# bindingflare/bling

Measured on AMD Instinct MI355X. Metric: Mrays/sec (primary+secondary), cornell-box 1024x1024 64spp at 1/2/4/8 GPU, higher is better.
Workload: dtype f32

## Files before the change

bling_amd/_ffi.py:

```python
from __future__ import annotations

import ctypes as C
import os

_HERE = os.path.dirname(os.path.abspath(__file__))
LIBDIR = os.path.join(_HERE, "_lib")

c_f32p = C.POINTER(C.c_float)
c_u32p = C.POINTER(C.c_uint32)


PASS_TRAVERSAL_STATS = 1
PASS_KERNEL_TIMING = 2
PASS_TILE_IMAGES = 4
PASS_REGION_EVENTS = 8
PASS_NO_MIS_CULL = 16


class PassParams(C.Structure):
    _fields_ = [("seed", C.c_uint32), ("pass_index", C.c_uint32), ("shard_rank", C.c_int32),
                ("shard_world", C.c_int32), ("tile_stride", C.c_int32), ("chunk_paths", C.c_int32),
                ("flags", C.c_uint32), ("tiles_device", C.c_void_p), ("tiles_capacity", C.c_uint64)]


# ... 67 lines not shown
        lib.bling_host_summary.restype = C.c_char_p
        lib.bling_host_free.argtypes = [C.c_void_p]
        lib.bling_host_config.argtypes = [C.c_void_p, C.POINTER(RenderConfig)]
        lib.bling_host_filter_size.argtypes = [C.c_void_p, c_f32p]
        lib.bling_host_filter_table.argtypes = [C.c_void_p, c_f32p]
        lib.bling_host_counts.argtypes = [C.c_void_p, c_u32p]
        lib.bling_host_last_error.restype = C.c_char_p
        lib.bling_host_film_to_rgb.argtypes = [c_f32p, C.c_int, C.c_int, c_f32p]
        lib.bling_host_film_splat_to_rgb.argtypes = [c_f32p, c_f32p, C.c_float, C.c_int, C.c_int, c_f32p]
        lib.bling_host_light.argtypes = [C.c_void_p, C.POINTER(LightTracer)]
        lib.bling_host_write_hdr.argtypes = [C.c_char_p, c_f32p, C.c_int, C.c_int]
        lib.bling_host_write_hdr.restype = C.c_int
        lib.bling_host_rgb_pixels.argtypes = [c_f32p, C.c_int, C.c_int, C.POINTER(C.c_uint8)]
        lib.bling_host_write_png.argtypes = [C.c_char_p, c_f32p, C.c_int, C.c_int]
        lib.bling_host_write_png.restype = C.c_int
        _host = lib
    return _host


HIP_SYMBOLS = ["bling_create", "bling_scene_upload", "bling_scene_validate", "bling_render_pass", "bling_render_pass_device",
               "bling_trace", "bling_trace_device", "bling_sample_li", "bling_sample_li_vertices", "bling_pass_tile_layout",
               "bling_film_add_tiles", "bling_film_add_shards", "bling_sppm_pass", "bling_sppm_pixel_stats", "bling_sppm_reset",
               "bling_render", "bling_debug_stream_bytes", "bling_debug_scene_info", "bling_debug_mis_culled", "bling_debug_set_mis_cull", "bling_debug_sppm_hitpoints", "bling_debug_sppm_buckets",
               "bling_light_pass", "bling_debug_light_records", "bling_destroy", "bling_last_error", "bling_version"]


class Progress(C.Structure):
    _fields_ = [("kind", C.c_int32), ("pass_", C.c_int32), ("film", C.POINTER(C.c_float)), ("splat_weight", C.c_float),
                ("pass_stats", C.POINTER(Stats)), ("region", C.c_int32 * 4)]


PROGRESS_STARTED, PROGRESS_SAMPLES_ADDED, PROGRESS_REGION_STARTED, PROGRESS_PASS_DONE = 0, 1, 2, 3
ProgressFn = C.CFUNCTYPE(C.c_int, C.c_void_p, C.POINTER(Progress))
STREAM_NAMES = "queue,hit,meta,org,dir,mdir,mhit,occ,fac,cf,T,L,Tn,lsc,bsc,sh_o,sh_d,result,qflag".split(",")


def hip() -> C.CDLL:
    global _hip
    if _hip is None:
        var = os.environ.get("BLING_HIP_VARIANT", "")
        path = os.path.join(LIBDIR, f"libbling_hip_{var}.so" if var else "libbling_hip.so")
        if not os.path.exists(path):
            raise OSError(f"{path} missing: run `make` (the HIP core has no CPU fallback)")
        lib = C.CDLL(path)
        lib.bling_create.argtypes = [C.POINTER(C.c_int), C.c_int, C.POINTER(C.c_void_p)]
        lib.bling_create.restype = C.c_int
        lib.bling_scene_upload.argtypes = [C.c_void_p, C.c_void_p]
        lib.bling_scene_upload.restype = C.c_int
        if hasattr(lib, "bling_scene_validate"):
            lib.bling_scene_validate.argtypes = [C.c_void_p]
            lib.bling_scene_validate.restype = C.c_int
        lib.bling_render_pass.argtypes = [C.c_void_p, C.POINTER(PassParams), c_f32p, C.POINTER(Stats)]
        lib.bling_render_pass.restype = C.c_int
        lib.bling_render_pass_device.argtypes = [C.c_void_p, C.POINTER(PassParams), C.c_void_p, C.POINTER(Stats)]
        lib.bling_render_pass_device.restype = C.c_int
        lib.bling_pass_tile_layout.argtypes = [C.c_void_p, C.POINTER(PassParams), C.POINTER(C.c_int32),
                                               C.POINTER(C.c_size_t), C.POINTER(C.c_int32), C.POINTER(C.c_int32)]
        lib.bling_pass_tile_layout.restype = C.c_int
        lib.bling_film_add_tiles.argtypes = [C.c_void_p, C.POINTER(PassParams), C.c_void_p, C.c_void_p]
        lib.bling_film_add_tiles.restype = C.c_int
        lib.bling_film_add_shards.argtypes = [C.c_void_p, C.POINTER(PassParams), C.POINTER(C.c_void_p), C.c_void_p]
        lib.bling_film_add_shards.restype = C.c_int
        lib.bling_trace.argtypes = [C.c_void_p, c_f32p, C.c_size_t, C.c_int, c_f32p, c_u32p, c_f32p]
        lib.bling_trace.restype = C.c_int
        lib.bling_trace_device.argtypes = [C.c_void_p, C.c_void_p, C.c_size_t, C.c_int, C.c_void_p, C.c_void_p,
                                           C.c_void_p, C.c_int, C.POINTER(C.c_double)]
        lib.bling_trace_device.restype = C.c_int
# ... 46 lines not shown
```

bling_amd/csrc/core/core_internal.h:

```cpp
#pragma once
#include <hip/hip_runtime.h>

#include <algorithm>
#include <type_traits>
#include <cstdio>
#include <cstring>
#include <memory>
#include <stdexcept>
#include <string>
#include <vector>

#include "../../../include/bling.h"
#include "../common/scene_features.h"
#include "bvh_build.h"
#include "wavefront.h"
#include "sppm.h"
#include "light_tracer.h"

namespace bcore {
using namespace bd;

struct HipError : std::runtime_error { using std::runtime_error::runtime_error; };

#define HIPCHK(x)                                                                        \
  do {                                                                                   \
    hipError_t e_ = (x);                                                                 \
    if (e_ != hipSuccess) throw HipError(std::string(#x) + ": " + hipGetErrorString(e_)); \
  } while (0)

template <class T>
struct DBuf {
  T* p = nullptr;
  size_t n = 0;
  DBuf() = default;
  DBuf(const DBuf&) = delete;
  DBuf& operator=(const DBuf&) = delete;
  void alloc(size_t count) {
    free();
    if (count == 0) return;
    HIPCHK(hipMalloc(&p, count * sizeof(T)));
    n = count;
  }
  void upload(const T* h, size_t count) {
    alloc(count);
    if (count) HIPCHK(hipMemcpy(p, h, count * sizeof(T), hipMemcpyHostToDevice));
  }
  void free() { if (p) { (void)hipFree(p); p = nullptr; n = 0; } }
  ~DBuf() { free(); }
};


constexpr uint64_t kSetBytes = 9 * 16 + 8 + 4 + 64 + 64;
constexpr uint64_t kSetSpectraBytes = 3 * 64;
constexpr uint64_t kPathFixedBytes = 16 + 8 + 6 * 4 + 1 + 4 + 2 * 4;
constexpr uint64_t kDlSlotBytes = 16 + 16 + 64;
constexpr int kMaxDlDepth = 16;

struct SppmState {
  bool ready = false;
  uint32_t hp_cap = 0, items_cap = 0, n_stats = 0, nth = 0, n_tiles = 0, n_ext = 0;
  DBuf<float4> hp_pos, hp_hit, hp_o, hp_d, hp_f, result;
  DBuf<Bsdf> hp_bsdf;
  DBuf<float2> img;
  DBuf<uint32_t> hp_count, cnt, bstart, bcur, items;
  DBuf<float> r2, nacc, splat, film, kd_mr, kd_c;
  DBuf<unsigned long long> hp_key;
  DBuf<SppmGrid> grid;
  DBuf<unsigned long long> ctr;
  DBuf<TileDesc> tiles;
  void free_all() {
    for (auto* b : {&hp_pos, &hp_hit, &hp_o, &hp_d, &hp_f, &result}) b->free();
    img.free(); hp_bsdf.free();
    for (auto* b : {&hp_count, &cnt, &bstart, &bcur, &items}) b->free();
    for (auto* b : {&r2, &nacc, &splat, &film, &kd_mr, &kd_c}) b->free();
    hp_key.free(); grid.free(); ctr.free(); tiles.free();
    ready = false; hp_cap = items_cap = 0;
  }
};

struct LightState {
  DBuf<float> splat;
  DBuf<unsigned long long> ctr;
  DBuf<uint4> rec;
  DBuf<uint32_t> rec_count;
  void free_all() { splat.free(); ctr.free(); rec.free(); rec_count.free(); }
};

}

using namespace bd;
using namespace bcore;

struct bling_ctx {
  using WaveState = bd::WaveState;
  int device = 0;
  hipStream_t stream = nullptr;
  bool has_scene = false;
  DevScene S{};
  DBuf<float4> nodes, tri_geo, pkt;
  DBuf<float4> leaf_geo;
  DBuf<uint32_t> refs;
  DBuf<float> tri_normals;
  DBuf<float4> tri_frame;
  DBuf<uint8_t> tri_has_n;
  DBuf<int32_t> tri_material, tri_prim, shape_prim;
  DBuf<DevShape> shapes;
  DBuf<bling_material> materials;
  DBuf<bling_texture> textures;
  DBuf<bling_scalar_texture> stex;
  DBuf<bling_light> lights;
  DBuf<bling_image> images;
  std::vector<std::unique_ptr<DBuf<float>>> light_arrays;
  uint32_t cap = 0;
  struct SetBufs {
    DBuf<float4> org, dir, hit, mdir, fac, cf, sh_o, sh_d, T, Tn, L, lsc, bsc;
    DBuf<uint4> meta;
    DBuf<float2> mhit;
    DBuf<uint32_t> occ;
    void alloc(uint32_t n, bool spectra) {
      for (auto* b : {&org, &dir, &hit, &mdir, &fac, &cf, &sh_o, &sh_d}) b->alloc(n);
      meta.alloc(n); mhit.alloc(n); occ.alloc(n);
      T.alloc((size_t)4 * n); L.alloc((size_t)4 * n);
      if (spectra) { Tn.alloc((size_t)4 * n); lsc.alloc((size_t)4 * n); bsc.alloc((size_t)4 * n); }
      else { Tn.free(); lsc.free(); bsc.free(); }
    }
    void free() {
      for (auto* b : {&org, &dir, &hit, &mdir, &fac, &cf, &sh_o, &sh_d, &T, &Tn, &L, &lsc, &bsc}) b->free();
      meta.free(); mhit.free(); occ.free();
    }
    PathSet view() const {
      return PathSet{org.p, dir.p, hit.p, meta.p, mdir.p, mhit.p, occ.p, fac.p, cf.p, sh_o.p, sh_d.p,
                     T.p, Tn.p, L.p, lsc.p, bsc.p};
    }
  } set[2];
  bool sets_spectra = false, sets_two = false;
  DBuf<float4> corg, dl_org, dl_dir, dl_T;
  DBuf<uint32_t> dl_mask;
  int dl_levels = 0;
  DBuf<float4> result;
  DBuf<float2> img;
  DBuf<uint32_t> qmem, qcount, blk;
  DBuf<float> march;
  DBuf<uint8_t> qflag;
  DBuf<TileDesc> tiles_dev;
  DBuf<Counters> counters;
  uint64_t mis_culled = 0;
  bool mis_cull_ok = false;
  bool mis_cull_off = false;
  uint64_t stream_bytes[2 * BLING_N_STREAMS] = {};
  DBuf<DevScene> dscene;
  DBuf<float> film_dev;
  DBuf<float> tr_rays, tr_t, tr_bary;
  DBuf<uint32_t> tr_prim;
  int bvh_depth = 0, bvh_leaves = 0, bvh_max_leaf = 0, bvh4_depth = 0;
  uint32_t num_prims = 0;
  uint32_t features = FT_ALL;
  size_t lds_trace = 0;
  bool lds_all = false;
  size_t lds_trace4 = 0;
  bool lds_all4 = false;
  DBuf<float4> nodes4;
  DBuf<int32_t> stack4_ovf;
  bling_render_config cfg{};
  SppmState sppm;
// ... 142 lines not shown
```

bling_amd/csrc/core/wavefront.h:

```cpp
#pragma once
#include "../../../include/bling.h"
#include "dev_shade.h"
#include "dev_trace.h"

namespace bd {

constexpr int kSkyWaves = 3;
#ifndef BLING_CORNELL_SHADE_WAVES
#define BLING_CORNELL_SHADE_WAVES 4
#endif
template <uint32_t F>
constexpr int shade_min_waves() {
  return ((F & FT_ENV_SKY) && (F & FT_GLASS) && !(F & (FT_TRIS | FT_SUBSTRATE | FT_BUMP))) ? kSkyWaves
       : ((F & (FT_GLASS | FT_SUBSTRATE | FT_BUMP)) ? 2
       : (F == (FT_MATTE | FT_AREA | FT_TRIS) ? BLING_CORNELL_SHADE_WAVES : ((F & FT_TRIS) ? 3 : 1)));
}
#define SHADE_OCC __attribute__((amdgpu_waves_per_eu(shade_min_waves<F>(), 8)))
#ifndef BLING_ALLL_WAVES
#define BLING_ALLL_WAVES 8
#endif
template <uint32_t F, bool ALLL>
constexpr int trace_min_waves() { return (F & FT_FRACTAL) ? 3 : ((ALLL && use_bvh4<F>()) ? BLING_ALLL_WAVES : 1); }
#define TRACE_OCC __attribute__((amdgpu_waves_per_eu(trace_min_waves<F, ALLL>(), 8)))

constexpr uint32_t VF_SH = 1u, VF_MIS = 2u, VF_TERM = 4u;
constexpr uint32_t VF_SPEC = 8u;
DEV uint32_t vf_depth(uint32_t vf) { return (vf >> 4) & 31u; }
DEV int vf_intl(uint32_t vf) { return (int)((vf >> 16) & 0xFFu) - 1; }
DEV int vf_light(uint32_t vf) { return (int)(vf >> 24); }
DEV uint32_t vf_make(int intl, int depth) { return ((uint32_t)(intl + 1) & 0xFFu) << 16 | ((uint32_t)depth & 31u) << 4; }
constexpr uint32_t ENTRY_CONT = 0u, ENTRY_MIS = 1u;

enum QueueId : int { Q_SHADE0 = 0, Q_SHADE1 = 1, Q_CLOSEST = 2, Q_ANY = 3, Q_RESOLVE = 4, Q_N = 5 };

struct PathSet {
  float4 *org, *dir, *hit;
  uint4* meta;
  float4* mdir;
  float2* mhit;
  uint32_t* occ;
  float4 *fac, *cf, *sh_o, *sh_d;
  float4 *T, *Tn, *L, *lsc, *bsc;
};

struct Est { float4 mdir, fac, cf; float2 mhit; uint32_t occ; };
DEV Est load_est(const PathSet& P, uint32_t s, uint32_t vf, bool factored_) {
  Est m;
  m.mdir = P.mdir[s];
  m.mhit = (vf & 2u) ? P.mhit[s] : make_float2(0.f, 0.f);
  m.occ = (vf & 1u) ? P.occ[s] : 0u;
  m.fac = factored_ ? P.fac[s] : make_float4(0.f, 0.f, 0.f, 0.f);
  m.cf = factored_ ? P.cf[s] : make_float4(0.f, 0.f, 0.f, 0.f);
  return m;
}
DEV Est load_est_eager(const PathSet& P, uint32_t s, bool factored_) {
  Est m;
  m.mdir = P.mdir[s];
  m.mhit = P.mhit[s];
  m.occ = P.occ[s];
  m.fac = factored_ ? P.fac[s] : make_float4(0.f, 0.f, 0.f, 0.f);
  m.cf = factored_ ? P.cf[s] : make_float4(0.f, 0.f, 0.f, 0.f);
  return m;
}

struct WaveState {
  PathSet cur;
  PathSet nxt;
  float4* corg;
  float2* img;
  float4* result;
  float4* Lfull;
  float* dbg;
  float* march_t;
  uint32_t* queue[Q_N];
  uint32_t* qcount;
  uint8_t* qflag;
  uint32_t* blk;
  unsigned long long* sb;
  float4* dl_org;
  float4* dl_dir;
  float4* dl_T;
  uint32_t* dl_mask;
  uint32_t cap;
  uint32_t mis_cull;
};

#ifndef BLING_DEBUG_VERTEX
#define BLING_DEBUG_VERTEX 0
#endif
#if BLING_DEBUG_VERTEX
#define DVREC(W, i, d, f, v) \
  do { if ((W).dbg && (d) >= 0 && (d) < BLING_DV_DEPTHS) (W).dbg[((size_t)(i) * BLING_DV_DEPTHS + (d)) * BLING_DV_FIELDS + (f)] = (v); } while (0)
#else
#define DVREC(W, i, d, f, v) do { } while (0)
#endif
#define DVREC3(W, i, d, f, v) do { DVREC(W, i, d, f, (v).x); DVREC(W, i, d, (f) + 1, (v).y); DVREC(W, i, d, (f) + 2, (v).z); } while (0)

constexpr uint32_t QF_RESOLVE = 1u, QF_ANY = 2u, QF_MIS = 4u, QF_CONT = 8u, QF_MISCULL = 16u;
constexpr int QF_COUNTS = 5;
constexpr int QC_MISCULL = 5, QC_N = 6;
constexpr uint32_t COMPACT_CHUNK = 4096;

struct Counters {
  unsigned long long cam, cont, mis, shadow, dropped, node_visits, tri_tests, shape_tests, vertices, march_ticks;
  unsigned long long c_node_visits, c_tri_tests, c_shape_tests, c_march_ticks;
  unsigned long long mis_culled;
  unsigned long long sb[2 * BLING_N_STREAMS];
};

#ifndef BLING_STREAM_STATS
#define BLING_STREAM_STATS 0
#endif
enum StreamId : int { SB_QUEUE, SB_HIT, SB_META, SB_ORG, SB_DIR, SB_MDIR, SB_MHIT, SB_OCC, SB_FAC, SB_CF, SB_T, SB_L,
                      SB_TN, SB_LSC, SB_BSC, SB_SHO, SB_SHD, SB_RESULT, SB_QFLAG };
static_assert(SB_QFLAG + 1 == BLING_N_STREAMS, "stream list of include/bling.h");
DEV void sb_count(unsigned long long* sb, int k, bool wr, uint32_t bytes, bool pred) {
#if BLING_STREAM_STATS
  const unsigned long long m = __ballot(pred);
  const uint32_t lead = (uint32_t)__ffsll((long long)__ballot(1)) - 1u;
  if (m && sb && (threadIdx.x & 63u) == lead) atomicAdd(&sb[2 * k + (wr ? 1 : 0)], (unsigned long long)__popcll(m) * bytes);
#else
  (void)sb; (void)k; (void)wr; (void)bytes; (void)pred;
#endif
}
#define SBR(W, k, bytes, pred) sb_count((W).sb, (k), false, (bytes), (pred))
#define SBW(W, k, bytes, pred) sb_count((W).sb, (k), true, (bytes), (pred))

DEV uint32_t wave_append(uint32_t* counter, bool pred) {
  unsigned long long mask = __ballot(pred);
  if (!pred) return 0u;
  uint32_t lane = threadIdx.x & 63u;
  uint32_t leader = (uint32_t)__ffsll((long long)mask) - 1u;
  uint32_t base = 0u;
  if (lane == leader) base = atomicAdd(counter, (uint32_t)__popcll(mask));
  base = __shfl(base, (int)leader, 64);
  return base + (uint32_t)__popcll(mask & ((1ull << lane) - 1ull));
}

DEV void store_sp(float4* dst, uint32_t i, const Sp& s) {
  float4* p = dst + 4 * (size_t)i;
#pragma unroll
  for (int q = 0; q < 4; ++q) p[q] = make_float4(s.v[4 * q], s.v[4 * q + 1], s.v[4 * q + 2], s.v[4 * q + 3]);
}
DEV Sp load_sp(const float4* src, uint32_t i) {
  const float4* p = src + 4 * (size_t)i;
  Sp s;
// ... 514 lines not shown
      float fm = 0.f, fs1 = 0.f, fs2 = 0.f, wpdf = 0.f;
      {
        float lb1, lb2; rnd2(S, k, db2, &lb1, &lb2);
        float s; V3 bwi;
        const float bpdf = sample_bsdf_diffuse1<F>(bsdf, wo, lb1, lb2, s, bwi);
        DVREC3(W, sid, dvd, 18, bwi); DVREC(W, sid, dvd, 21, bpdf);
        const bool cand = !(bpdf == 0.f) && !is_black(diffuse1_f(r, s));
        mis_culled = cand && mis_cull_test<F>(S, W, Lt, p, bwi, eps, bpdf, fabsf(s) < INFINITY);
        if (cand && !mis_culled) {
          const float lpdf = light_pdf<F>(S, Lt, p, bwi);
          m.mdir = make_float4(bwi.x, bwi.y, bwi.z,
                               kd_flag_w(power_heuristic(bpdf, lpdf), kd_root(S, Ray{p, bwi, eps, INFINITY})));
          fm = s;
          vf |= VF_MIS;
          app_mis = true;
        }
      }
      {
        float ld1, ld2; rnd2(S, k, dl2, &ld1, &ld2);
        LightSample smp = light_sample<F>(S, Lt, p, bsdf.cs.n, eps, ld1, ld2);
        DVREC3(W, sid, dvd, 14, smp.wi); DVREC(W, sid, dvd, 17, smp.pdf);
        float s1, s2;
        if (!(smp.pdf == 0.f) && !is_black(smp.li) && eval_bsdf_diffuse1<F>(bsdf, wo, smp.wi, s1, s2) &&
            !is_black(diffuse1_e(r, s1, s2))) {
          const float w = smp.delta ? 1.f : power_heuristic(smp.pdf, bsdf_pdf<F>(bsdf, wo, smp.wi));
          wpdf = w / smp.pdf; fs1 = s1; fs2 = s2;
          const float stmin = kd_root(S, smp.ray) ? smp.ray.tmin : INFINITY;
          O.sh_o[o] = make_float4(smp.ray.o.x, smp.ray.o.y, smp.ray.o.z, stmin);
          O.sh_d[o] = make_float4(smp.ray.d.x, smp.ray.d.y, smp.ray.d.z, smp.ray.tmax);
          vf |= VF_SH;
          app_sh = true;
        }
      }
      m.fac = make_float4(fm, fs1, fs2, wpdf);
      return;
    }
    {
      float lBc = rnd1(S, k, db1);
      float lb1, lb2; rnd2(S, k, db2, &lb1, &lb2);
      Sp bf; V3 bwi; int bfl;
      float bpdf = sample_bsdf<F>(bsdf, wo, lBc, lb1, lb2, bf, bwi, bfl);
      DVREC3(W, sid, dvd, 18, bwi); DVREC(W, sid, dvd, 21, bpdf);
      const bool cand = !(bpdf == 0.f) && !is_black(bf);
      mis_culled = cand && mis_cull_test<F>(S, W, Lt, p, bwi, eps, bpdf, !s_bad(bf));
      if (cand && !mis_culled) {
        float lpdf = light_pdf<F>(S, Lt, p, bwi);
        float w = power_heuristic(bpdf, lpdf);
        store_sp(O.bsc, o, bf);
        m.mdir = make_float4(bwi.x, bwi.y, bwi.z, kd_flag_w(w, kd_root(S, Ray{p, bwi, eps, INFINITY})));
        vf |= VF_MIS;
        app_mis = true;
      }
    }
    {
      float ld1, ld2; rnd2(S, k, dl2, &ld1, &ld2);
      LightSample smp = light_sample<F>(S, Lt, p, bsdf.cs.n, eps, ld1, ld2);
      DVREC3(W, sid, dvd, 14, smp.wi); DVREC(W, sid, dvd, 17, smp.pdf);
      if (!(smp.pdf == 0.f) && !is_black(smp.li)) {
        float dps[2] = {__builtin_nanf(""), __builtin_nanf("")};
        Sp f = eval_bsdf<F>(bsdf, wo, smp.wi, dps);
        if (!is_black(f)) {
          float w = smp.delta ? 1.f : power_heuristic(smp.pdf, bsdf_pdf<F>(bsdf, wo, smp.wi, dps));
          store_sp(O.lsc, o, sscale(f * smp.li, w / smp.pdf));
          O.sh_o[o] = make_float4(smp.ray.o.x, smp.ray.o.y, smp.ray.o.z, kd_root(S, smp.ray) ? smp.ray.tmin : INFINITY);
          O.sh_d[o] = make_float4(smp.ray.d.x, smp.ray.d.y, smp.ray.d.z, smp.ray.tmax);
          vf |= VF_SH;
          app_sh = true;
// ... 33 lines not shown
    LC c = coordinate_system(nn);
    dgg.p = pp; dgg.n = nn; dgg.u = 0.f; dgg.v = 0.f; dgg.dpdu = c.s; dgg.dpdv = c.t;
    eps = S.fractal.epsilon * 2.f;
    mat = S.fractal.material;
  }
  dgs = dgg;
  if ((F & FT_TRI_NORMALS) && kind == REF_TRI && S.tri_normals && S.tri_has_n[idx]) {
    const float* nn = gen(S.tri_normals) + 9 * idx;
    float b1 = hv.z, b2 = hv.w, b0 = 1.f - b1 - b2;
    V3 nsp = sm(b0, mk(nn[0], nn[1], nn[2])) + sm(b1, mk(nn[3], nn[4], nn[5])) + sm(b2, mk(nn[6], nn[7], nn[8]));
    V3 ns = normalize(nsp);
    V3 ssp = normalize(dgg.dpdu);
    V3 tsp = cross(ssp, ns);
    if (sqlen(tsp) > 0.f) { dgs.dpdu = cross(normalize(tsp), ns); dgs.dpdv = normalize(tsp); }
    else { LC c = coordinate_system(ns); dgs.dpdu = c.s; dgs.dpdv = c.t; }
    dgs.n = ns;
  }
}

template <uint32_t F>
DEV Sp resolve_L(const DevScene& S, const WaveState& W, uint32_t s, uint32_t vf, const Est& m, const Sp& T0,
                 bool first, uint32_t sid, int dvd, const float4& o) {
  (void)sid;
  int lc = S.num_lights;
  Sp ld = sconst(0.f);
  if (lc > 0) {
    Sp ls = sconst(0.f), bs = sconst(0.f);
    const int ln = vf_light(vf);
    float4 fc = make_float4(0.f, 0.f, 0.f, 0.f);
    const float* rf = nullptr;
    if constexpr (factored<F>()) {
      if (vf & (VF_SH | VF_MIS)) {
        fc = m.fac;
        rf = lobe_r(S, __float_as_uint(m.cf.z));
      }
      if ((vf & VF_SH) && m.occ == 0u)
        ls = sscale(diffuse1_e(rf, fc.y, fc.z) * sload(light_rec<F>(S, ln).radiance), fc.w);
    } else {
      if ((vf & VF_SH) && m.occ == 0u) ls = load_sp(W.cur.lsc, s);
      SBR(W, SB_LSC, 64, (vf & VF_SH) && m.occ == 0u);
    }
    if (vf & VF_SH) DVREC(W, sid, dvd, 28, m.occ ? 1.f : 0.f);
    if (vf & VF_MIS) {
      const bling_light& Lt = light_rec<F>(S, ln);
      const uint32_t ref = __float_as_uint(m.mhit.y);
      const float4 d = m.mdir;
      V3 wi = mk(d.x, d.y, d.z);
      DVREC(W, sid, dvd, 29, ref == REF_NONE ? INFINITY : m.mhit.x);
      if (ref == REF_NONE) {
        const Sp bf = factored<F>() ? diffuse1_f(rf, fc.x) : load_sp(W.cur.bsc, s);
        SBR(W, SB_BSC, 64, !factored<F>());
        bs = sscale(bf * light_le<F>(Lt, wi), fabsf(d.w));
      } else if ((ref >> 30) == REF_SHAPE) {
        const DevShape& hs = gen(S.shapes[ref & 0x3FFFFFFFu]);
        SBR(W, SB_BSC, 64, !factored<F>() && hs.light == ln);
        if (hs.light == ln) {
          DG dg = shape_dg<F>(hs, Ray{mk(o.x, o.y, o.z), wi, o.w, INFINITY}, m.mhit.x);
          Sp le = dot(dg.n, -wi) > 0.f ? sload(gen(S.lights[ln]).radiance) : sconst(0.f);
          const Sp bf = factored<F>() ? diffuse1_f(rf, fc.x) : load_sp(W.cur.bsc, s);
          bs = sscale(bf * le, fabsf(d.w));
        }
      }
    }
    ld = ls + bs;
    if (lc > 1) ld = sscale(ld, (float)lc);
  }
  const int il = vf_intl(vf);
  Sp lhere = (il >= 0 ? sload(light_rec<F>(S, il).radiance) : sconst(0.f)) + ld;
  const Sp L0 = first ? sconst(0.f) : load_sp(W.cur.L, s);
#if BLING_DEBUG_VERTEX
  {
    const Sp Lr = L0 + T0 * lhere;
    float a = 0.f, b = 0.f;
    for (int q = 0; q < 16; ++q) { a += lhere.v[q]; b += Lr.v[q]; }
    DVREC(W, sid, dvd, 30, a); DVREC(W, sid, dvd, 31, b);
  }
#endif
  return L0 + T0 * lhere;
}

template <uint32_t F>
DEV Sp next_throughput(const DevScene& S, const PathSet& P, uint32_t s, const float4 cf, const Sp& Tv, float pc) {
  if constexpr (factored<F>()) {
    (void)pc;
    const Sp f = diffuse1_f(lobe_r(S, __float_as_uint(cf.z)), cf.x);
    return sscale(f * Tv, 1.f / cf.y);
  } else {
    (void)cf;
    return sscale(load_sp(P.Tn, s) * Tv, 1.f / pc);
  }
}

template <uint32_t F>
DEV uint32_t shade_vertex(const DevScene& S, const WaveState& W, const PathSet& O, uint32_t o, int depth, uint32_t seed,
                          uint32_t pass, float ty, uint32_t vfin, float4 hv, const Ray& ray, uint32_t pix,
                          uint32_t nid, uint32_t sid) {
  const bool spec = (vfin & VF_SPEC) != 0;
  bool app_sh = false, app_mis = false, app_cont = false, mis_culled = false;
  SampleKey k = sample_key(seed, pass, pix, nid);
  DG dgg, dgs;
  float eps;
  int mat, hit_light;
  hit_geometry<F>(S, ray, hv, dgg, dgs, eps, mat, hit_light);
  DVREC3(W, sid, depth, 0, ray.o); DVREC3(W, sid, depth, 3, ray.d); DVREC(W, sid, depth, 6, hv.x);
  DVREC3(W, sid, depth, 10, dgg.n); DVREC(W, sid, depth, 13, eps);
  int intl_light = (spec && hit_light >= 0 && dot(dgg.n, ray.d) > 0.f) ? hit_light : -1;
  float ttmp[(F & FT_PROCTEX) ? 32 : 1];
  Bsdf bsdf = make_bsdf<F>(S, mat, dgg, dgs, ttmp);
  V3 wo = -ray.d;
  V3 p = bsdf.p;
  DVREC3(W, sid, depth, 7, p);
  uint32_t vf = vf_make(intl_light, 0);
  Est m;
  m.mdir = make_float4(0.f, 0.f, 0.f, 0.f);
  m.fac = make_float4(0.f, 0.f, 0.f, 0.f);
  const float* r = (factored<F>() && bsdf.n) ? bsdf.b[0].r : nullptr;
  const uint32_t rtex = r ? (uint32_t)((const char*)r - (const char*)gen(S.textures)) : ~0u;
  float pc = depth <= 7 ? 1.f : hmin(0.75f, ty);
  float x = rnd1(S, k, 3 + 4 * depth);
  DVREC(W, sid, depth, 26, pc); DVREC(W, sid, depth, 27, x);
  bool cont = !(x > pc);
  float s1c = 0.f;
  V3 cwi = mk(0.f, 0.f, 0.f);
  if (cont) {
    float uc = rnd1(S, k, 0 + 4 * depth);
    float ud1, ud2; rnd2(S, k, 0 + 3 * depth, &ud1, &ud2);
    int cfl = F_REFL | F_DIFF;
    float cpdf;
    if constexpr (factored<F>()) {
      (void)uc;
      cpdf = sample_bsdf_diffuse1<F>(bsdf, wo, ud1, ud2, s1c, cwi);
      cont = !(cpdf == 0.f || is_black(diffuse1_f(r, s1c)));
    } else {
      Sp cf;
      cpdf = sample_bsdf<F>(bsdf, wo, uc, ud1, ud2, cf, cwi, cfl);
      cont = !(cpdf == 0.f || is_black(cf));
      if (cont) store_sp(O.Tn, o, cf);
      SBW(W, SB_TN, 64, cont);
    }
    DVREC3(W, sid, depth, 22, cwi); DVREC(W, sid, depth, 25, cpdf);
    if (cont) {
      if ((cfl & F_SPEC) == F_SPEC) vf |= VF_SPEC;
      app_cont = true;
    }
  }
  if (!cont) vf |= VF_TERM;
  if constexpr (factored<F>()) O.cf[o] = make_float4(s1c, pc, __uint_as_float(rtex), 0.f);
  O.org[o] = make_float4(p.x, p.y, p.z, eps);
  O.dir[o] = make_float4(cwi.x, cwi.y, cwi.z, kd_flag_w(pc, !cont || kd_root(S, Ray{p, cwi, eps, INFINITY})));
  direct_setup<F>(S, W, O, o, k, bsdf, wo, p, eps, 1 + 4 * depth, 1 + 3 * depth, 2 + 4 * depth, 2 + 3 * depth, vf,
                  app_mis, app_sh, mis_culled, m, sid, depth);
  if (app_mis) O.mdir[o] = m.mdir;
  if constexpr (factored<F>()) O.fac[o] = m.fac;
  O.meta[o] = make_uint4(vf, pix, nid, sid);
  SBW(W, SB_CF, 16, factored<F>() && (app_cont || app_sh || app_mis));
  SBW(W, SB_ORG, 16, app_cont || app_mis);
  SBW(W, SB_DIR, 16, app_cont);
  SBW(W, SB_MDIR, 16, app_mis);
  SBW(W, SB_FAC, 16, factored<F>() && (app_sh || app_mis));
  SBW(W, SB_META, 16, true);
  SBW(W, SB_SHO, 16, app_sh);
  SBW(W, SB_SHD, 16, app_sh);
  SBW(W, SB_LSC, 64, !factored<F>() && app_sh);
  SBW(W, SB_BSC, 64, !factored<F>() && app_mis);
  return QF_RESOLVE | (app_sh ? QF_ANY : 0u) | (app_mis ? QF_MIS : 0u) | (app_cont ? QF_CONT : 0u) |
         (mis_culled ? QF_MISCULL : 0u);
}

template <uint32_t F>
DEV void shade_end(const DevScene& S, const WaveState& W, uint32_t sid, const Sp& T, bool spec_miss, V3 rd, Sp L,
                   unsigned long long& n_drop) {
  if (spec_miss) {
    Sp sum = sconst(0.f);
#if !defined(BLING_SKY_COST_EXPERIMENT)
    for (int l = 0; l < S.num_lights; ++l) sum = sum + light_le<F>(gen(S.lights[l]), rd);
#endif
    L = L + T * sum;
  }
  finalize(W, sid, L, n_drop);
}

constexpr uint32_t SHADE_RING = 128;
template <uint32_t F, bool FUSED>
static __global__ __launch_bounds__(256) SHADE_OCC void k_shade(const DevScene* __restrict__ Sptr, WaveState W, int depth, int qin,
                                               uint32_t seed, uint32_t pass, Counters* __restrict__ C) {
  const DevScene& S = *Sptr;
  const uint32_t n = *(volatile uint32_t*)&W.qcount[qin];
  const uint32_t* q = W.queue[qin];
  unsigned long long n_drop = 0;
  __shared__ uint32_t ring_e[4][SHADE_RING];
  __shared__ float ring_y[4][SHADE_RING];
  __shared__ float4 ring_h[4][SHADE_RING];
// ... 15 lines not shown
  uint32_t qnext = 0u;
  {
    const uint32_t e0 = (blockIdx.x * (blockDim.x >> 6) + wv) * 64u + lane;
    if (e0 < n) qnext = q[e0];
  }
  uint32_t base = (blockIdx.x * (blockDim.x >> 6) + wv) * 64u;
  for (;;) {
    const bool more = base < n;
    if (more) {
      const uint32_t e = base + lane;
      const uint32_t qcur = qnext;
      if (e + nwaves * 64u < n) qnext = q[e + nwaves * 64u];
      bool vert = false;
      uint32_t s = 0u;
      float ty = 0.f;
      float4 hv = make_float4(0.f, 0.f, 0.f, 0.f), ro = hv, rdv = hv;
      uint4 meta = make_uint4(0u, 0u, 0u, 0u);
      if (e < n) {
        s = qcur;
        hv = W.cur.hit[s];
        meta = W.cur.meta[s];
        ro = W.cur.org[s];
        rdv = W.cur.dir[s];
        vert = !(FUSED && (meta.x & VF_TERM)) && __float_as_uint(hv.y) != REF_NONE && depth != S.max_depth;
      }
      const unsigned long long msk = __ballot(vert);
      const uint32_t nv = (uint32_t)__popcll(msk);
      const uint32_t o = base + (uint32_t)__popcll(msk & below);
      if (e < n) {
        if (lane >= nv) W.qflag[base + lane] = 0u;
        Sp L = sconst(0.f);
        bool ends = false;
        Est m;
        m.cf = make_float4(0.f, 0.f, 0.f, 0.f);
        Sp Tp = sconst(1.f);
        if constexpr (FUSED) {
          m = load_est_eager(W.cur, s, factored<F>());
          if (depth > 1) Tp = load_sp(W.cur.T, s);
          L = resolve_L<F>(S, W, s, meta.x, m, Tp, depth == 1, meta.w, depth - 1, ro);
          SBR(W, SB_MDIR, 16, (meta.x & VF_MIS) != 0u);
          SBR(W, SB_MHIT, 8, (meta.x & VF_MIS) != 0u);
          SBR(W, SB_OCC, 4, (meta.x & VF_SH) != 0u);
          SBR(W, SB_FAC, 16, factored<F>() && (meta.x & (VF_SH | VF_MIS)) != 0u);
          SBR(W, SB_T, 64, depth > 1);
          SBR(W, SB_L, 64, depth > 1);
          if (meta.x & VF_TERM) { finalize(W, meta.w, L, n_drop); ends = true; }
        }
        if (!ends) {
          const uint32_t ref = __float_as_uint(hv.y);
          const bool spec_miss = ref == REF_NONE && (meta.x & VF_SPEC) != 0;
          const bool hit = ref != REF_NONE && depth != S.max_depth;
          Sp Td = sconst(1.f);
          if (FUSED && (hit || spec_miss)) Td = next_throughput<F>(S, W.cur, s, m.cf, Tp, fabsf(rdv.w));
          SBR(W, SB_TN, 64, FUSED && !factored<F>() && (hit || spec_miss));
          SBR(W, SB_CF, 16, FUSED && factored<F>() && ((hit || spec_miss) || (meta.x & (VF_SH | VF_MIS)) != 0u));
          SBR(W, SB_DIR, 16, hit || spec_miss);
          SBR(W, SB_ORG, 16, hit || (FUSED && (meta.x & VF_MIS) != 0u && __float_as_uint(m.mhit.y) != REF_NONE &&
                                     (__float_as_uint(m.mhit.y) >> 30) == REF_SHAPE));
          SBW(W, SB_L, 64, FUSED && hit);
          SBW(W, SB_T, 64, FUSED && hit);
          if (hit) {
            if constexpr (FUSED) {
              store_sp(W.nxt.L, o, L);
              store_sp(W.nxt.T, o, Td);
            }
            if (depth > 7) ty = sY(Td);
          } else {
            shade_end<F>(S, W, meta.w, Td, spec_miss, mk(rdv.x, rdv.y, rdv.z), L, n_drop);
          }
        }
        SBR(W, SB_QUEUE, 4, true);
        SBR(W, SB_HIT, 16, true);
        SBR(W, SB_META, 16, true);
        SBW(W, SB_QFLAG, 1, true);
      }
      if (vert) {
        const uint32_t slot = (head + cnt + (uint32_t)__popcll(msk & below)) & (SHADE_RING - 1u);
        ring_e[wv][slot] = o; ring_y[wv][slot] = ty;
        ring_h[wv][slot] = hv; ring_m[wv][slot] = meta;
        ring_o[wv][slot] = ro; ring_d[wv][slot] = rdv;
      }
      cnt += (uint32_t)__popcll(msk);
      __builtin_amdgcn_fence(__ATOMIC_RELEASE, "wavefront");
      __builtin_amdgcn_wave_barrier();
      __builtin_amdgcn_fence(__ATOMIC_ACQUIRE, "wavefront");
      base += nwaves * 64u;
    }
    if (cnt >= 64u || (!more && cnt > 0u)) {
      const uint32_t take = cnt < 64u ? cnt : 64u;
      if (lane < take) shade_from_ring((head + lane) & (SHADE_RING - 1u));
      head = (head + take) & (SHADE_RING - 1u);
      cnt -= take;
    }
    if (!more && cnt == 0u) break;
  }
  flush_dropped(C, n_drop);
}

template <uint32_t F>
static __global__ __launch_bounds__(256) SHADE_OCC void k_shade_dl(const DevScene* __restrict__ Sptr, WaveState W, int qin, uint32_t seed,
                                                  uint32_t pass, Counters* __restrict__ C) {
  const DevScene& S = *Sptr;
  const uint32_t n = *(volatile uint32_t*)&W.qcount[qin];
  const uint32_t* q = W.queue[qin];
  unsigned long long n_drop = 0;
  const size_t cap = W.cap;
  const PathSet& P = W.cur;
  for (uint32_t e = blockIdx.x * blockDim.x + threadIdx.x; e < n; e += gridDim.x * blockDim.x) {
    const uint32_t i = q[e];
    const uint4 meta = P.meta[i];
    const int d = (int)vf_depth(meta.x);
    const float4 hv = P.hit[i], ro = W.corg[i], rdv = P.dir[i];
    const Ray ray{mk(ro.x, ro.y, ro.z), mk(rdv.x, rdv.y, rdv.z), ro.w, INFINITY};
    const bool hit = __float_as_uint(hv.y) != REF_NONE;
    bool app_sh = false, app_mis = false, mis_culled = false, next = false;
    uint32_t mask = W.dl_mask[i], vf = 0u;
    float4 no = ro, nd = rdv;
    int nlev = 0;
    if (hit) {
      const Sp T = load_sp(P.T, i);
      SampleKey k = sample_key(seed, pass, meta.y, meta.z);
      DG dgg, dgs;
      float eps;
      int mat, hit_light;
      hit_geometry<F>(S, ray, hv, dgg, dgs, eps, mat, hit_light);
      const V3 wo = -ray.d;
      const int intl = (hit_light >= 0 && dot(dgg.n, wo) > 0.f) ? hit_light : -1;
      float ttmp[(F & FT_PROCTEX) ? 32 : 1];
      Bsdf bsdf = make_bsdf<F>(S, mat, dgg, dgs, ttmp);
      const V3 p = bsdf.p;
      vf = vf_make(intl, 0);
      Est m;
      m.mdir = make_float4(0.f, 0.f, 0.f, 0.f);
      m.fac = make_float4(0.f, 0.f, 0.f, 0.f);
      const float* lr = (factored<F>() && bsdf.n) ? bsdf.b[0].r : nullptr;
      const uint32_t rtex = lr ? (uint32_t)((const char*)lr - (const char*)gen(S.textures)) : ~0u;
      direct_setup<F>(S, W, P, i, k, bsdf, wo, p, eps, 2 * d, 2 * d, 1 + 2 * d, 1 + 2 * d, vf, app_mis, app_sh, mis_culled, m, i);
      if (app_mis) P.mdir[i] = m.mdir;
      if constexpr (factored<F>()) { P.fac[i] = m.fac; P.cf[i] = make_float4(0.f, 1.f, __uint_as_float(rtex), 0.f); }
      if (d + 1 != S.max_depth) {
        Sp fr, ft; V3 wr, wt;
        const bool hr = !(sample_bsdf_spec<F>(bsdf, wo, F_REFL, fr, wr) == 0.f);
        const bool ht = !(sample_bsdf_spec<F>(bsdf, wo, F_TRANS, ft, wt) == 0.f);
        const float4 po = make_float4(p.x, p.y, p.z, eps);
        if (hr) {
          next = true; no = po; nd = make_float4(wr.x, wr.y, wr.z, 0.f); nlev = d + 1;
          store_sp(P.Tn, i, fr * T);
        }
        if (ht) {
          if (hr) {
            const size_t slot = (size_t)(d + 1) * cap + i;
            W.dl_org[slot] = po;
            W.dl_dir[slot] = make_float4(wt.x, wt.y, wt.z, 0.f);
            store_sp(W.dl_T + 4 * (size_t)(d + 1) * cap, i, ft * T);
            mask |= 1u << (d + 1);
          } else {
            next = true; no = po; nd = make_float4(wt.x, wt.y, wt.z, 0.f); nlev = d + 1;
            store_sp(P.Tn, i, ft * T);
          }
        }
      }
      P.org[i] = make_float4(p.x, p.y, p.z, eps);
    }
    if (!next && mask != 0u) {
      const int j = 31 - __clz(mask);
      const size_t slot = (size_t)j * cap + i;
      mask &= ~(1u << j);
      next = true; no = W.dl_org[slot]; nd = W.dl_dir[slot]; nlev = j;
      store_sp(P.Tn, i, load_sp(W.dl_T + 4 * (size_t)j * cap, i));
    }
    W.dl_mask[i] = mask;
    if (next) {
// ... 367 lines not shown
```

include/bling.h:

```cpp
#ifndef BLING_H
#define BLING_H

#include <stddef.h>
#include <stdint.h>
#include "bling_scene.h"

#ifdef __cplusplus
extern "C" {
#endif

#define BLING_OK           0
#define BLING_EINVAL      -1
#define BLING_ENODEV      -2
#define BLING_EHIP        -3
#define BLING_ENOSCENE    -4
#define BLING_EUNSUPPORTED -5
#define BLING_ENOMEM      -6

#define BLING_MISS 0xFFFFFFFFu

typedef struct bling_ctx bling_ctx;

typedef struct bling_pass_params {
    uint32_t seed;
// ... 99 lines not shown

int bling_sppm_pass(bling_ctx* ctx, uint32_t seed, uint32_t pass_index, float* film_out, float* splat_out,
                    bling_sppm_stats* stats);

int bling_sppm_pixel_stats(bling_ctx* ctx, float* r2_out, float* n_out, size_t* n_pixels);

int bling_sppm_reset(bling_ctx* ctx);

int bling_debug_sppm_hitpoints(bling_ctx* ctx, float* pos_r2, uint64_t* keys, size_t cap, size_t* n);
int bling_debug_sppm_buckets(bling_ctx* ctx, uint32_t* bstart, uint32_t* items, float* mr, size_t cap_b,
                             size_t cap_i, size_t* nb, size_t* ni);

typedef struct bling_light_stats {
    uint64_t photons;
    uint64_t photon_rays;
    uint64_t shadow_rays;
    uint64_t splats;
    uint64_t dropped;
    double   ms_total;
} bling_light_stats;

int bling_light_pass(bling_ctx* ctx, uint32_t seed, uint32_t pass_index, float* splat_inout,
                     bling_light_stats* stats);

typedef struct bling_light_record {
    uint32_t photon, depth;
    int32_t  sx, sy;
    float    x, y, z;
    uint32_t pad;
} bling_light_record;
int bling_debug_light_records(bling_ctx* ctx, uint32_t seed, uint32_t pass_index, uint32_t first_photon,
                              uint32_t n_photons, bling_light_record* records, size_t cap, size_t* n);

#define BLING_STREAM_NAMES "queue,hit,meta,org,dir,mdir,mhit,occ,fac,cf,T,L,Tn,lsc,bsc,sh_o,sh_d,result,qflag"
#define BLING_N_STREAMS 19
int bling_debug_stream_bytes(bling_ctx* ctx, uint64_t* out, size_t n, size_t* n_streams);

int bling_debug_mis_culled(bling_ctx* ctx, uint64_t* out);
int bling_debug_set_mis_cull(bling_ctx* ctx, int on);

int bling_debug_scene_info(bling_ctx* ctx, char* buf, size_t size, size_t* len);

void bling_destroy(bling_ctx* ctx);

const char* bling_last_error(void);

const char* bling_version(void);

#ifdef __cplusplus
}
#endif
#endif
```

Before: 13230.

## Repack factored path streams: split fm and rtex, drop cf buffer, lazy MIS loads

Replaces the per-path 16-byte cf stream with a 4-byte rtex texture offset and moves the MIS lobe factor into a separate 4-byte fm stream. The continuation coefficient now lives in fac.x and the continuation pdf comes from the direction's w component. MIS direction and hit data are read only when the MIS flag is set, for matte/area/tri scenes with culling on. The goal is fewer bytes of global memory traffic per path vertex, at the cost of one extra buffer and a bit more bookkeeping.

```diff
diff --git a/bling_amd/_ffi.py b/bling_amd/_ffi.py
--- a/bling_amd/_ffi.py
+++ b/bling_amd/_ffi.py
@@ -123,7 +123,7 @@
 
 PROGRESS_STARTED, PROGRESS_SAMPLES_ADDED, PROGRESS_REGION_STARTED, PROGRESS_PASS_DONE = 0, 1, 2, 3
 ProgressFn = C.CFUNCTYPE(C.c_int, C.c_void_p, C.POINTER(Progress))
-STREAM_NAMES = "queue,hit,meta,org,dir,mdir,mhit,occ,fac,cf,T,L,Tn,lsc,bsc,sh_o,sh_d,result,qflag".split(",")
+STREAM_NAMES = "queue,hit,meta,org,dir,mdir,mhit,fm,occ,fac,rtex,T,L,Tn,lsc,bsc,sh_o,sh_d,result,qflag".split(",")
 
 
 def hip() -> C.CDLL:
diff --git a/bling_amd/csrc/core/core_internal.h b/bling_amd/csrc/core/core_internal.h
--- a/bling_amd/csrc/core/core_internal.h
+++ b/bling_amd/csrc/core/core_internal.h
@@ -50,7 +50,7 @@
 };
 
 
-constexpr uint64_t kSetBytes = 9 * 16 + 8 + 4 + 64 + 64;
+constexpr uint64_t kSetBytes = 8 * 16 + 8 + 3 * 4 + 64 + 64;
 constexpr uint64_t kSetSpectraBytes = 3 * 64;
 constexpr uint64_t kPathFixedBytes = 16 + 8 + 6 * 4 + 1 + 4 + 2 * 4;
 constexpr uint64_t kDlSlotBytes = 16 + 16 + 64;
@@ -113,23 +113,24 @@
   std::vector<std::unique_ptr<DBuf<float>>> light_arrays;
   uint32_t cap = 0;
   struct SetBufs {
-    DBuf<float4> org, dir, hit, mdir, fac, cf, sh_o, sh_d, T, Tn, L, lsc, bsc;
+    DBuf<float4> org, dir, hit, mdir, fac, sh_o, sh_d, T, Tn, L, lsc, bsc;
     DBuf<uint4> meta;
     DBuf<float2> mhit;
-    DBuf<uint32_t> occ;
+    DBuf<float> fm;
+    DBuf<uint32_t> occ, rtex;
     void alloc(uint32_t n, bool spectra) {
-      for (auto* b : {&org, &dir, &hit, &mdir, &fac, &cf, &sh_o, &sh_d}) b->alloc(n);
-      meta.alloc(n); mhit.alloc(n); occ.alloc(n);
+      for (auto* b : {&org, &dir, &hit, &mdir, &fac, &sh_o, &sh_d}) b->alloc(n);
+      meta.alloc(n); mhit.alloc(n); fm.alloc(n); occ.alloc(n); rtex.alloc(n);
       T.alloc((size_t)4 * n); L.alloc((size_t)4 * n);
       if (spectra) { Tn.alloc((size_t)4 * n); lsc.alloc((size_t)4 * n); bsc.alloc((size_t)4 * n); }
       else { Tn.free(); lsc.free(); bsc.free(); }
     }
     void free() {
-      for (auto* b : {&org, &dir, &hit, &mdir, &fac, &cf, &sh_o, &sh_d, &T, &Tn, &L, &lsc, &bsc}) b->free();
-      meta.free(); mhit.free(); occ.free();
+      for (auto* b : {&org, &dir, &hit, &mdir, &fac, &sh_o, &sh_d, &T, &Tn, &L, &lsc, &bsc}) b->free();
+      meta.free(); mhit.free(); fm.free(); occ.free(); rtex.free();
     }
     PathSet view() const {
-      return PathSet{org.p, dir.p, hit.p, meta.p, mdir.p, mhit.p, occ.p, fac.p, cf.p, sh_o.p, sh_d.p,
+      return PathSet{org.p, dir.p, hit.p, meta.p, mdir.p, mhit.p, fm.p, occ.p, fac.p, rtex.p, sh_o.p, sh_d.p,
                      T.p, Tn.p, L.p, lsc.p, bsc.p};
     }
   } set[2];
diff --git a/bling_amd/csrc/core/wavefront.h b/bling_amd/csrc/core/wavefront.h
--- a/bling_amd/csrc/core/wavefront.h
+++ b/bling_amd/csrc/core/wavefront.h
@@ -38,29 +38,37 @@
   uint4* meta;
   float4* mdir;
   float2* mhit;
+  float* fm;
   uint32_t* occ;
-  float4 *fac, *cf, *sh_o, *sh_d;
+  float4* fac;
+  uint32_t* rtex;
+  float4 *sh_o, *sh_d;
   float4 *T, *Tn, *L, *lsc, *bsc;
 };
 
-struct Est { float4 mdir, fac, cf; float2 mhit; uint32_t occ; };
+struct Est { float4 mdir, fac; float2 mhit; uint32_t occ; float fm; uint32_t rtex; };
 DEV Est load_est(const PathSet& P, uint32_t s, uint32_t vf, bool factored_) {
   Est m;
   m.mdir = P.mdir[s];
   m.mhit = (vf & 2u) ? P.mhit[s] : make_float2(0.f, 0.f);
   m.occ = (vf & 1u) ? P.occ[s] : 0u;
   m.fac = factored_ ? P.fac[s] : make_float4(0.f, 0.f, 0.f, 0.f);
-  m.cf = factored_ ? P.cf[s] : make_float4(0.f, 0.f, 0.f, 0.f);
+  m.fm = (factored_ && (vf & 2u)) ? P.fm[s] : 0.f;
+  m.rtex = factored_ ? P.rtex[s] : ~0u;
   return m;
 }
-DEV Est load_est_eager(const PathSet& P, uint32_t s, bool factored_) {
-  Est m;
-  m.mdir = P.mdir[s];
-  m.mhit = P.mhit[s];
+template <uint32_t F>
+constexpr bool mis_lazy() { return (F & ~(FT_MATTE | FT_AREA | FT_TRIS)) == 0; }
+DEV void load_est_fused(Est& m, const PathSet& P, uint32_t s, bool factored_) {
   m.occ = P.occ[s];
   m.fac = factored_ ? P.fac[s] : make_float4(0.f, 0.f, 0.f, 0.f);
-  m.cf = factored_ ? P.cf[s] : make_float4(0.f, 0.f, 0.f, 0.f);
-  return m;
+  m.rtex = factored_ ? P.rtex[s] : ~0u;
+}
+DEV void load_est_mis(Est& m, const PathSet& P, uint32_t s, uint32_t vf, bool factored_, bool lazy) {
+  const bool mis = !lazy || (vf & VF_MIS) != 0u;
+  m.mdir = mis ? P.mdir[s] : make_float4(0.f, 0.f, 0.f, 0.f);
+  m.mhit = mis ? P.mhit[s] : make_float2(0.f, 0.f);
+  m.fm = (factored_ && (vf & VF_MIS) != 0u) ? P.fm[s] : 0.f;
 }
 
 struct WaveState {
@@ -111,7 +119,7 @@
 #ifndef BLING_STREAM_STATS
 #define BLING_STREAM_STATS 0
 #endif
-enum StreamId : int { SB_QUEUE, SB_HIT, SB_META, SB_ORG, SB_DIR, SB_MDIR, SB_MHIT, SB_OCC, SB_FAC, SB_CF, SB_T, SB_L,
+enum StreamId : int { SB_QUEUE, SB_HIT, SB_META, SB_ORG, SB_DIR, SB_MDIR, SB_MHIT, SB_FM, SB_OCC, SB_FAC, SB_RTEX, SB_T, SB_L,
                       SB_TN, SB_LSC, SB_BSC, SB_SHO, SB_SHD, SB_RESULT, SB_QFLAG };
 static_assert(SB_QFLAG + 1 == BLING_N_STREAMS, "stream list of include/bling.h");
 DEV void sb_count(unsigned long long* sb, int k, bool wr, uint32_t bytes, bool pred) {
@@ -692,7 +700,8 @@
           app_sh = true;
         }
       }
-      m.fac = make_float4(fm, fs1, fs2, wpdf);
+      m.fm = fm;
+      m.fac.y = fs1; m.fac.z = fs2; m.fac.w = wpdf;
       return;
     }
     {
@@ -792,7 +801,7 @@
     if constexpr (factored<F>()) {
       if (vf & (VF_SH | VF_MIS)) {
         fc = m.fac;
-        rf = lobe_r(S, __float_as_uint(m.cf.z));
+        rf = lobe_r(S, m.rtex);
       }
       if ((vf & VF_SH) && m.occ == 0u)
         ls = sscale(diffuse1_e(rf, fc.y, fc.z) * sload(light_rec<F>(S, ln).radiance), fc.w);
@@ -808,7 +817,7 @@
       V3 wi = mk(d.x, d.y, d.z);
       DVREC(W, sid, dvd, 29, ref == REF_NONE ? INFINITY : m.mhit.x);
       if (ref == REF_NONE) {
-        const Sp bf = factored<F>() ? diffuse1_f(rf, fc.x) : load_sp(W.cur.bsc, s);
+        const Sp bf = factored<F>() ? diffuse1_f(rf, m.fm) : load_sp(W.cur.bsc, s);
         SBR(W, SB_BSC, 64, !factored<F>());
         bs = sscale(bf * light_le<F>(Lt, wi), fabsf(d.w));
       } else if ((ref >> 30) == REF_SHAPE) {
@@ -817,7 +826,7 @@
         if (hs.light == ln) {
           DG dg = shape_dg<F>(hs, Ray{mk(o.x, o.y, o.z), wi, o.w, INFINITY}, m.mhit.x);
           Sp le = dot(dg.n, -wi) > 0.f ? sload(gen(S.lights[ln]).radiance) : sconst(0.f);
-          const Sp bf = factored<F>() ? diffuse1_f(rf, fc.x) : load_sp(W.cur.bsc, s);
+          const Sp bf = factored<F>() ? diffuse1_f(rf, m.fm) : load_sp(W.cur.bsc, s);
           bs = sscale(bf * le, fabsf(d.w));
         }
       }
@@ -840,13 +849,12 @@
 }
 
 template <uint32_t F>
-DEV Sp next_throughput(const DevScene& S, const PathSet& P, uint32_t s, const float4 cf, const Sp& Tv, float pc) {
+DEV Sp next_throughput(const DevScene& S, const PathSet& P, uint32_t s, const Est& m, const Sp& Tv, float pc) {
   if constexpr (factored<F>()) {
-    (void)pc;
-    const Sp f = diffuse1_f(lobe_r(S, __float_as_uint(cf.z)), cf.x);
-    return sscale(f * Tv, 1.f / cf.y);
+    const Sp f = diffuse1_f(lobe_r(S, m.rtex), m.fac.x);
+    return sscale(f * Tv, 1.f / pc);
   } else {
-    (void)cf;
+    (void)m;
     return sscale(load_sp(P.Tn, s) * Tv, 1.f / pc);
   }
 }
@@ -874,6 +882,7 @@
   Est m;
   m.mdir = make_float4(0.f, 0.f, 0.f, 0.f);
   m.fac = make_float4(0.f, 0.f, 0.f, 0.f);
+  m.fm = 0.f;
   const float* r = (factored<F>() && bsdf.n) ? bsdf.b[0].r : nullptr;
   const uint32_t rtex = r ? (uint32_t)((const char*)r - (const char*)gen(S.textures)) : ~0u;
   float pc = depth <= 7 ? 1.f : hmin(0.75f, ty);
@@ -905,19 +914,23 @@
     }
   }
   if (!cont) vf |= VF_TERM;
-  if constexpr (factored<F>()) O.cf[o] = make_float4(s1c, pc, __uint_as_float(rtex), 0.f);
+  if constexpr (factored<F>()) { O.rtex[o] = rtex; m.fac.x = s1c; }
   O.org[o] = make_float4(p.x, p.y, p.z, eps);
   O.dir[o] = make_float4(cwi.x, cwi.y, cwi.z, kd_flag_w(pc, !cont || kd_root(S, Ray{p, cwi, eps, INFINITY})));
   direct_setup<F>(S, W, O, o, k, bsdf, wo, p, eps, 1 + 4 * depth, 1 + 3 * depth, 2 + 4 * depth, 2 + 3 * depth, vf,
                   app_mis, app_sh, mis_culled, m, sid, depth);
-  if (app_mis) O.mdir[o] = m.mdir;
+  if (app_mis) {
+    O.mdir[o] = m.mdir;
+    if constexpr (factored<F>()) O.fm[o] = m.fm;
+  }
   if constexpr (factored<F>()) O.fac[o] = m.fac;
   O.meta[o] = make_uint4(vf, pix, nid, sid);
-  SBW(W, SB_CF, 16, factored<F>() && (app_cont || app_sh || app_mis));
+  SBW(W, SB_FAC, 16, factored<F>() && (app_cont || app_sh || app_mis));
+  SBW(W, SB_RTEX, 4, factored<F>() && (app_cont || app_sh || app_mis));
   SBW(W, SB_ORG, 16, app_cont || app_mis);
   SBW(W, SB_DIR, 16, app_cont);
   SBW(W, SB_MDIR, 16, app_mis);
-  SBW(W, SB_FAC, 16, factored<F>() && (app_sh || app_mis));
+  SBW(W, SB_FM, 4, factored<F>() && app_mis);
   SBW(W, SB_META, 16, true);
   SBW(W, SB_SHO, 16, app_sh);
   SBW(W, SB_SHD, 16, app_sh);
@@ -999,16 +1012,18 @@
         Sp L = sconst(0.f);
         bool ends = false;
         Est m;
-        m.cf = make_float4(0.f, 0.f, 0.f, 0.f);
+        m.fac = make_float4(0.f, 0.f, 0.f, 0.f);
+        m.rtex = ~0u;
         Sp Tp = sconst(1.f);
         if constexpr (FUSED) {
-          m = load_est_eager(W.cur, s, factored<F>());
+          load_est_fused(m, W.cur, s, factored<F>());
           if (depth > 1) Tp = load_sp(W.cur.T, s);
+          load_est_mis(m, W.cur, s, meta.x, factored<F>(), mis_lazy<F>() && W.mis_cull != 0u);
           L = resolve_L<F>(S, W, s, meta.x, m, Tp, depth == 1, meta.w, depth - 1, ro);
           SBR(W, SB_MDIR, 16, (meta.x & VF_MIS) != 0u);
           SBR(W, SB_MHIT, 8, (meta.x & VF_MIS) != 0u);
           SBR(W, SB_OCC, 4, (meta.x & VF_SH) != 0u);
-          SBR(W, SB_FAC, 16, factored<F>() && (meta.x & (VF_SH | VF_MIS)) != 0u);
+          SBR(W, SB_FM, 4, factored<F>() && (meta.x & VF_MIS) != 0u);
           SBR(W, SB_T, 64, depth > 1);
           SBR(W, SB_L, 64, depth > 1);
           if (meta.x & VF_TERM) { finalize(W, meta.w, L, n_drop); ends = true; }
@@ -1018,9 +1033,8 @@
           const bool spec_miss = ref == REF_NONE && (meta.x & VF_SPEC) != 0;
           const bool hit = ref != REF_NONE && depth != S.max_depth;
           Sp Td = sconst(1.f);
-          if (FUSED && (hit || spec_miss)) Td = next_throughput<F>(S, W.cur, s, m.cf, Tp, fabsf(rdv.w));
+          if (FUSED && (hit || spec_miss)) Td = next_throughput<F>(S, W.cur, s, m, Tp, fabsf(rdv.w));
           SBR(W, SB_TN, 64, FUSED && !factored<F>() && (hit || spec_miss));
-          SBR(W, SB_CF, 16, FUSED && factored<F>() && ((hit || spec_miss) || (meta.x & (VF_SH | VF_MIS)) != 0u));
           SBR(W, SB_DIR, 16, hit || spec_miss);
           SBR(W, SB_ORG, 16, hit || (FUSED && (meta.x & VF_MIS) != 0u && __float_as_uint(m.mhit.y) != REF_NONE &&
                                      (__float_as_uint(m.mhit.y) >> 30) == REF_SHAPE));
@@ -1035,6 +1049,13 @@
           } else {
             shade_end<F>(S, W, meta.w, Td, spec_miss, mk(rdv.x, rdv.y, rdv.z), L, n_drop);
           }
+        }
+        {
+          const uint32_t ref = __float_as_uint(hv.y);
+          const bool goes_on = !ends && ((ref != REF_NONE && depth != S.max_depth) || (ref == REF_NONE && (meta.x & VF_SPEC) != 0));
+          const bool need = FUSED && factored<F>() && (goes_on || (meta.x & (VF_SH | VF_MIS)) != 0u);
+          SBR(W, SB_FAC, 16, need);
+          SBR(W, SB_RTEX, 4, need);
         }
         SBR(W, SB_QUEUE, 4, true);
         SBR(W, SB_HIT, 16, true);
@@ -1100,11 +1121,15 @@
       Est m;
       m.mdir = make_float4(0.f, 0.f, 0.f, 0.f);
       m.fac = make_float4(0.f, 0.f, 0.f, 0.f);
+      m.fm = 0.f;
       const float* lr = (factored<F>() && bsdf.n) ? bsdf.b[0].r : nullptr;
       const uint32_t rtex = lr ? (uint32_t)((const char*)lr - (const char*)gen(S.textures)) : ~0u;
       direct_setup<F>(S, W, P, i, k, bsdf, wo, p, eps, 2 * d, 2 * d, 1 + 2 * d, 1 + 2 * d, vf, app_mis, app_sh, mis_culled, m, i);
-      if (app_mis) P.mdir[i] = m.mdir;
-      if constexpr (factored<F>()) { P.fac[i] = m.fac; P.cf[i] = make_float4(0.f, 1.f, __uint_as_float(rtex), 0.f); }
+      if (app_mis) {
+        P.mdir[i] = m.mdir;
+        if constexpr (factored<F>()) P.fm[i] = m.fm;
+      }
+      if constexpr (factored<F>()) { P.fac[i] = m.fac; P.rtex[i] = rtex; }
       if (d + 1 != S.max_depth) {
         Sp fr, ft; V3 wr, wt;
         const bool hr = !(sample_bsdf_spec<F>(bsdf, wo, F_REFL, fr, wr) == 0.f);
diff --git a/include/bling.h b/include/bling.h
--- a/include/bling.h
+++ b/include/bling.h
@@ -155,8 +155,8 @@
 int bling_debug_light_records(bling_ctx* ctx, uint32_t seed, uint32_t pass_index, uint32_t first_photon,
                               uint32_t n_photons, bling_light_record* records, size_t cap, size_t* n);
 
-#define BLING_STREAM_NAMES "queue,hit,meta,org,dir,mdir,mhit,occ,fac,cf,T,L,Tn,lsc,bsc,sh_o,sh_d,result,qflag"
-#define BLING_N_STREAMS 19
+#define BLING_STREAM_NAMES "queue,hit,meta,org,dir,mdir,mhit,fm,occ,fac,rtex,T,L,Tn,lsc,bsc,sh_o,sh_d,result,qflag"
+#define BLING_N_STREAMS 20
 int bling_debug_stream_bytes(bling_ctx* ctx, uint64_t* out, size_t n, size_t* n_streams);
 
 int bling_debug_mis_culled(bling_ctx* ctx, uint64_t* out);
```

Result: faster. 13520 (median of 6 runs) (+2.2%).
